# mauruszach/multimodal_diffusion

Hardware: AMD Instinct MI355X
Metric: denoising steps/sec @256x256 multimodal-cond batch=32 (higher is better)
Workload: dtype f32 via 3xbf16 split operands (6-term products, f32 accumulate; fp32-level error); 1 GPU; C3: 256x256 audio->video CFG denoising step (cond+null MMDiT d512 L8 H8 + noise head + DDIM), 384+37 tokens, batch 32 per GPU, DDIM 50 steps, guidance 3.5; global_batch=32, sampler_steps=50, parallelism=dp1, launch=eager, matmul=bf16x3, attn=default, cfg_halves=one stacked 2B batch, one stream

## Files before the change

multimodal_diffusion_amd/csrc/avd_common.h:

```cpp
#pragma once
#include <hip/hip_runtime.h>
#include <stdint.h>
#include <stdio.h>
#include <stdarg.h>
#include <atomic>

#include "../../include/avdiff_hip.h"

namespace avd {

int set_error(int code, const char* fmt, ...);

#define AVD_REQUIRE(cond, code, ...)                       \
    do {                                                   \
        if (!(cond)) return avd::set_error((code), __VA_ARGS__); \
    } while (0)

#define AVD_CHECK_LAUNCH(name)                                                          \
    do {                                                                                \
        hipError_t e__ = hipGetLastError();                                             \
        if (e__ != hipSuccess)                                                          \
            return avd::set_error(AVD_ELAUNCH, "%s: %s", (name), hipGetErrorString(e__)); \
    } while (0)

// ... 99 lines not shown
                if (fabsf(a) < __builtin_inff()) { h = (h & 0xffff8000u) | 0x7f7fu; ra = a - bf16_lo(h); } else ra = 0.f;
            }
            if ((h & 0x7fff0000u) == 0x7f800000u) {
                if (fabsf(b) < __builtin_inff()) { h = (h & 0x8000ffffu) | 0x7f7f0000u; rb = b - bf16_hi(h); } else rb = 0.f;
            }
        }
        const unsigned int m = pk_bf16(ra, rb);
        const float sa = ra - bf16_lo(m), sb = rb - bf16_hi(m);
        H[e] = h;
        Mi[e] = m;
        Lo[e] = pk_bf16(sa, sb);
    }
}

template <bool RANGE_CHECK = true>
__device__ __forceinline__ void store_split8(unsigned char* img, int64_t r, int k, int K, const float* v) {
    u32x4 H, Mi, Lo;
    split8<RANGE_CHECK>(v, H, Mi, Lo);
    const int rr = (int)(r & 127), half = (k >> 3) & 1;
    unsigned char* dst = img + ((r >> 7) * (K >> 4) + (k >> 4)) * (int64_t)S3_CHUNK + rr * 32 + ((half ^ ((rr >> 4) & 1)) << 4);
    *reinterpret_cast<u32x4*>(dst) = H;
    *reinterpret_cast<u32x4*>(dst + S3_PLANE) = Mi;
    *reinterpret_cast<u32x4*>(dst + 2 * S3_PLANE) = Lo;
}

typedef _Float16 f16x8 __attribute__((ext_vector_type(8)));
typedef _Float16 f16x2 __attribute__((ext_vector_type(2)));

__device__ __forceinline__ unsigned int pk_f16(float a, float b) {
    const f32x2 v = {a, b};
    return __builtin_bit_cast(unsigned int, __builtin_convertvector(v, f16x2));
}
__device__ __forceinline__ f32x2 unpk_f16(unsigned int p) { return __builtin_convertvector(__builtin_bit_cast(f16x2, p), f32x2); }

__device__ __forceinline__ void split8_h2(const float* v, float s, u32x4& H, u32x4& L) {
#pragma unroll
    for (int e = 0; e < 4; ++e) {
        const float a = v[2 * e] * s, b = v[2 * e + 1] * s;
        const unsigned int h = pk_f16(a, b);
        const f32x2 u = unpk_f16(h);
        H[e] = h;
        L[e] = pk_f16(a - u[0], b - u[1]);
    }
}
__device__ __forceinline__ void store_split8_h2(unsigned char* img, int64_t r, int k, int K, const float* v, float s) {
    u32x4 H, L;
// ... 72 lines not shown
extern int g_attn_pipe;
extern int g_s3_m16;
extern int g_s3_w128;
extern int g_s3_rt4;
extern int g_s3_deep4;
extern int g_s3_rt;
extern int g_vae_lat;
extern int g_vae_fold;
extern int g_codec_mfma;
extern int g_cfg_rows;
extern int g_s3_sn, g_s3_super4, g_s3_super8;
extern int g_s3_tile;
extern thread_local bool t_s3_two_streams;
int gemm_bf16x3_qkv3(const void* A3, const void* W3, const float* bias, void* img, int64_t M, int tokens, int heads, int K, float qscale,
                     int terms, hipStream_t st, float ab_scale = 1.f, float c_scale = 1.f, const float* ss_in = nullptr, float eps = 0.f);
int64_t qkv3_bytes(int B, int N, int H);
int64_t attn_fp8_ws_bytes(int B, int N, int H);
int attn_fp8(const void* qkv3, void* ws, int64_t ws_bytes, float* out, void* out3, int B, int N, int H, int n_query, hipStream_t st,
             int img_terms = 6, float img_scale = 1.f, float out_scale = 1.f);
int attn_bf16x3(const void* qkv3, float* out, void* out3, int B, int N, int H, int n_query, int terms, hipStream_t st,
                float img_scale = 1.f, float out_scale = 1.f, int out_tokens = 0);
int gemm_bf16x3(const void* A3, const void* W3, const float* bias, const float* R, float* C, void* C3, int64_t M, int N, int K,
                int act, int terms, hipStream_t st, float ab_scale = 1.f, float c_scale = 1.f, const float* ss_in = nullptr, float eps = 0.f,
                float* ss_out = nullptr, const float* gamma = nullptr, int r_seg = 0, int r_stride = 0);
bool gemm_bf16x3_resmap_supported(int terms);
bool gemm_bf16x3_rownorm_supported(int N, int terms);
extern int g_s3_splitk;
int gemm_bf16x3_splitk_slices(int64_t M, int N, int K, int terms);
int64_t gemm_bf16x3_splitk_ws_floats(int64_t M, int N, int ns);
constexpr int kS3SplitKMax = 4;
int64_t gemm_bf16x3_splitk_ws_max_floats(int64_t M, int N, int K);
int gemm_bf16x3_splitk(const void* A3, const void* W3, const float* bias, const float* R, float* C, void* C3, float* ss, int64_t M, int N,
                       int K, int terms, int ns, float* part, hipStream_t st);

}
```

multimodal_diffusion_amd/csrc/composite.hip:

```cpp
#include "avd_common.h"

#include <limits.h>
#include <stdlib.h>

#include <string.h>
#include <map>
#include <mutex>
#include <string>
#include <utility>
#include <vector>

namespace avd {

static thread_local char g_err[512] = "";

int set_error(int code, const char* fmt, ...) {
    va_list ap;
    va_start(ap, fmt);
    vsnprintf(g_err, sizeof(g_err), fmt, ap);
    va_end(ap);
    return code;
}

int LdsAttr::ensure(const void* kern, int lds_bytes, const char* what) {
// ... 119 lines not shown
    for (int l = 0; l < w->n_layers; ++l)
        if (!w->blocks[l].in_proj_weight3n || !w->blocks[l].fc1_weight3n) return false;
    return true;
}
static bool core_use_split_fold(const avd_core_weights* w) { return !g_no_fold && core_split_fold_capable(w); }

static bool core_split_rownorm_capable(const avd_core_weights* w) {
    return w->norm_kind == 0 && w->split_terms == 3 && gemm_bf16x3_rownorm_supported(w->d, 3);
}
static bool core_use_split_rownorm(const avd_core_weights* w) { return !g_no_fold && core_split_rownorm_capable(w); }

static bool core_use_fold(const avd_core_weights* w) {
    if (g_no_fold || w->norm_kind != 0) return false;
    if (!gemm_f32_fold_supported(3 * w->d, w->d) || !gemm_f32_fold_supported(w->d, w->d) ||
        !gemm_f32_fold_supported(w->mlp_hidden, w->d) || !gemm_f32_fold_supported(w->d, w->mlp_hidden))
        return false;
    for (int l = 0; l < w->n_layers; ++l)
        if (!w->blocks[l].in_proj_weight_n || !w->blocks[l].fc1_weight_n) return false;
    return true;
}

static int g_core_trim = 1;
static int64_t core_trim_floats(const avd_core_weights* w, int B, int N) { return (int64_t)B * N * w->d; }

static int64_t core_split_wide_bytes(const avd_core_weights* w, int B, int N) {
    const int64_t qkv3 = qkv3_bytes(B, N, w->n_heads), fc1 = split3_bytes((int64_t)B * N, w->mlp_hidden);
    return qkv3 > fc1 ? qkv3 : fc1;
}

static int64_t core_ws_bytes(const avd_core_weights* w, int B, int N) {
    const int64_t M = (int64_t)B * N;
    const int wide = 3 * w->d > w->mlp_hidden ? 3 * w->d : w->mlp_hidden;
    int64_t fp32_path = align_up(M * w->d * 4) + align_up(M * wide * 4) + 2 * align_up(M * (w->d / 32 + 1) * 4) +
                        align_up(gemm_f32_splitk_ws_max_floats(M, w->d, w->mlp_hidden) * 4);
    if (!core_split_capable(w, M)) return fp32_path;
    const int64_t wide_b = core_split_wide_bytes(w, B, N);
    const int64_t f8_b = w->attn_mode == 1 ? attn_fp8_ws_bytes(B, N, w->n_heads) : 0;
    const int64_t fold_b = core_split_fold_capable(w) ? align_up(split3_bytes(M, w->d)) + align_up(M * (w->d / 64) * 4)
                         : core_split_rownorm_capable(w) ? align_up(split3_bytes(M, w->d)) : 0;
    const int64_t sk_b = core_split_fold_capable(w) ? align_up(gemm_bf16x3_splitk_ws_max_floats(M, w->d, w->mlp_hidden) * 4) : 0;
    const int64_t trim_b = core_split_fold_capable(w) ? align_up(core_trim_floats(w, B, N) * 4) : 0;
    const int64_t split_path = align_up(wide_b) + align_up(split3_bytes(M, w->d)) + align_up(f8_b) + fold_b + sk_b + trim_b;
    return split_path > fp32_path ? split_path : fp32_path;
}

static int check_core(const avd_core_weights* w) {
    AVD_REQUIRE(w && w->blocks && w->final_norm_scale, AVD_EINVAL, "core: null weight table");
    AVD_REQUIRE(w->d > 0 && w->n_layers > 0 && w->n_heads > 0 && w->mlp_hidden > 0, AVD_EINVAL, "core: bad dims");
    AVD_REQUIRE(w->d % w->n_heads == 0, AVD_EINVAL, "core: d_model %d not divisible by n_heads %d", w->d, w->n_heads);
    AVD_REQUIRE(w->attn_mode == 0 || w->attn_mode == 1, AVD_EINVAL, "core: attn_mode must be 0 (follow the matmul mode) or 1 (fp8)");
    AVD_REQUIRE(w->norm_kind == 0 || w->norm_kind == 1, AVD_EINVAL, "core: norm_kind must be 0 (RMSNorm) or 1 (LayerNorm)");
    AVD_REQUIRE(w->d / w->n_heads == 64, AVD_EUNSUPPORTED, "core: head_dim %d unsupported (64 only)", w->d / w->n_heads);
    AVD_REQUIRE(w->d % 4 == 0 && w->mlp_hidden % 4 == 0, AVD_EUNSUPPORTED, "core: widths must be multiples of 4");
    AVD_REQUIRE(w->split_terms == 0 || w->split_terms == 6 || w->split_terms == 9 || w->split_terms == 1 || w->split_terms == 3, AVD_EINVAL,
                "core: split_terms must be 0/6 (default), 9 (strict), 1 (plain bf16) or 3 (f16x2), got %d", w->split_terms);
    if (w->split_terms == 3) {
        for (int l = 0; l < w->n_layers; ++l)
            for (int i = 0; i < 8; ++i) {
                const float s = w->blocks[l].f16x2_scale[i];
                AVD_REQUIRE(s > 0.f && s < __builtin_inff(), AVD_EINVAL, "core: blocks[%d].f16x2_scale[%d] must be positive and finite", l, i);
            }
    }
    return AVD_OK;
}
// ... 22 lines not shown
    const float scale = 1.0f / sqrtf((float)(d / H));
    const float* cur = x;
    AVD_REQUIRE(!(w->attn_mode == 1 && (kpm || w->norm_kind != 0)), AVD_EUNSUPPORTED,
                "core: attn_mode 1 (fp8 attention) cannot be combined with a key_padding_mask or norm_kind 1 (LayerNorm)");
    AVD_REQUIRE(!(w->attn_mode == 1 && !core_use_split(w, M)), AVD_EUNSUPPORTED,
                "core: attn_mode 1 (fp8 attention) reads the q|k|v image of the split-operand projections, which these weights / shapes "
                "do not take (every block needs its *_weight3 images; 3 d, d and mlp_hidden must be multiples of 256, d of 16)");
    if (!kpm && core_use_split(w, M)) {
        const int terms = w->split_terms;
        Carver cs{static_cast<char*>(ws), 0, ws_bytes};
        const int64_t wide_b = core_split_wide_bytes(w, B, N);
        float* qkv = cs.take((wide_b + 3) / 4);
        void* wide3 = qkv;
        void* hs = cs.take((split3_bytes(M, d) + 3) / 4);
        const int64_t f8_b = w->attn_mode == 1 ? attn_fp8_ws_bytes(B, N, H) : 0;
        float* f8w = cs.take((f8_b + 3) / 4);
        if (core_use_split_fold(w)) {
            void* hx = cs.take((split3_bytes(M, d) + 3) / 4);
            float* ss = cs.take(M * (d / 64));
            const int ns = gemm_bf16x3_splitk_slices(M, d, hid, terms);
            float* part = ns ? cs.take(gemm_bf16x3_splitk_ws_floats(M, d, ns)) : nullptr;
            const bool trim = g_core_trim && out_row0 == 0 && n_out_rows < N && w->attn_mode == 0 && gemm_bf16x3_resmap_supported(terms);
            float* yc = cs.take(core_trim_floats(w, B, N));
            const bool fused = g_mlp_fused && !ns && mlp_bf16x3_supported(d, hid, terms) && gemm_bf16x3_resmap_supported(terms);
            AVD_REQUIRE(cs.ok, AVD_EWORKSPACE, "core: workspace carve %lld > %lld bytes", (long long)cs.used, (long long)cs.cap);
            if (int rc = split3_rows_f32(cur, rd, hx, M, d, st, 0.f, ss)) return rc;
            for (int l = 0; l < w->n_layers; ++l) {
                const avd_block_weights& b = w->blocks[l];
                const bool last = l == w->n_layers - 1;
                const int nq = (last && out_row0 == 0) ? n_out_rows : N;
                if (last && trim) {
                    const int64_t Mc = (int64_t)B * nq;
                    if (int rc = gemm_bf16x3_qkv3(hx, b.in_proj_weight3n, b.in_proj_bias, qkv, M, N, H, d, scale * 1.4426950408889634f, terms, st,
                                                  1.f, 1.f, ss, w->norm_eps)) return rc;
                    if (int rc = attn_bf16x3(qkv, nullptr, hs, B, N, H, nq, terms, st, 1.f, 1.f, nq)) return rc;
                    if (int rc = gemm_bf16x3(hs, b.out_proj_weight3, b.out_proj_bias, cur, yc, hx, Mc, d, d, AVD_ACT_NONE, terms, st, 1.f, 1.f,
                                             nullptr, 0.f, ss, nullptr, nq, N)) return rc;
                    if (fused) {
                        if (int rc = mlp_bf16x3(hx, b.fc1_weight3n, b.fc1_bias, b.fc2_weight3, b.fc2_bias, ss, w->norm_eps, yc, yc, nullptr, nullptr, Mc,
                                                d, hid, st)) return rc;
                    } else {
                        if (int rc = gemm_bf16x3(hx, b.fc1_weight3n, b.fc1_bias, nullptr, nullptr, wide3, Mc, hid, d, AVD_ACT_GELU, terms, st, 1.f, 1.f,
                                                 ss, w->norm_eps)) return rc;
                        if (ns) {
                            if (int rc = gemm_bf16x3_splitk(wide3, b.fc2_weight3, b.fc2_bias, yc, yc, nullptr, nullptr, Mc, d, hid, terms, ns, part,
                                                            st)) return rc;
                        } else {
                            if (int rc = gemm_bf16x3(wide3, b.fc2_weight3, b.fc2_bias, yc, yc, nullptr, Mc, d, hid, AVD_ACT_NONE, terms, st)) return rc;
                        }
                    }
                    return rmsnorm_f32(yc, rd, w->final_norm_scale, y, RowMap{d, nq, (int64_t)N * d}, Mc, d, w->norm_eps, st);
                }
                if (int rc = gemm_bf16x3_qkv3(hx, b.in_proj_weight3n, b.in_proj_bias, qkv, M, N, H, d, scale * 1.4426950408889634f, terms, st,
                                              1.f, 1.f, ss, w->norm_eps)) return rc;
                if (w->attn_mode == 1) {
                    if (int rc = attn_fp8(qkv, f8w, f8_b, nullptr, hs, B, N, H, nq, st, terms, 1.f, 1.f)) return rc;
                } else {
                    if (int rc = attn_bf16x3(qkv, nullptr, hs, B, N, H, nq, terms, st, 1.f, 1.f)) return rc;
                }
                if (int rc = gemm_bf16x3(hs, b.out_proj_weight3, b.out_proj_bias, cur, y, hx, M, d, d, AVD_ACT_NONE, terms, st, 1.f, 1.f, nullptr,
                                         0.f, ss)) return rc;
                cur = y;
                if (fused) {
                    if (int rc = mlp_bf16x3(hx, b.fc1_weight3n, b.fc1_bias, b.fc2_weight3, b.fc2_bias, ss, w->norm_eps, y, y, last ? nullptr : hx,
                                            last ? nullptr : ss, M, d, hid, st)) return rc;
                    continue;
                }
                if (int rc = gemm_bf16x3(hx, b.fc1_weight3n, b.fc1_bias, nullptr, nullptr, wide3, M, hid, d, AVD_ACT_GELU, terms, st, 1.f, 1.f, ss,
                                         w->norm_eps)) return rc;
                if (ns) {
                    if (int rc = gemm_bf16x3_splitk(wide3, b.fc2_weight3, b.fc2_bias, y, y, last ? nullptr : hx, last ? nullptr : ss, M, d, hid,
                                                    terms, ns, part, st)) return rc;
                } else if (last) {
                    if (int rc = gemm_bf16x3(wide3, b.fc2_weight3, b.fc2_bias, y, y, nullptr, M, d, hid, AVD_ACT_NONE, terms, st)) return rc;
                } else {
                    if (int rc = gemm_bf16x3(wide3, b.fc2_weight3, b.fc2_bias, y, y, hx, M, d, hid, AVD_ACT_NONE, terms, st, 1.f, 1.f, nullptr, 0.f,
                                             ss)) return rc;
                }
            }
            return rmsnorm_f32(y, rd, w->final_norm_scale, y, rd, M, d, w->norm_eps, st);
        }
        const bool rown = core_use_split_rownorm(w);
        void* hn = rown ? cs.take((split3_bytes(M, d) + 3) / 4) : hs;
        AVD_REQUIRE(cs.ok, AVD_EWORKSPACE, "core: workspace carve %lld > %lld bytes", (long long)cs.used, (long long)cs.cap);
        for (int l = 0; l < w->n_layers; ++l) {
            const avd_block_weights& b = w->blocks[l];
            const bool last = l == w->n_layers - 1;
            const int nq = (last && out_row0 == 0) ? n_out_rows : N;
            const bool h2 = terms == 3;
            const float* fs = b.f16x2_scale;
            const float s_n1 = h2 ? fs[4] : 0.f, s_qkv = h2 ? fs[5] : 1.f, s_n2 = h2 ? fs[6] : 0.f, s_fc1 = h2 ? fs[7] : 1.f;
            const float w_in = h2 ? fs[0] : 1.f, w_out = h2 ? fs[1] : 1.f, w_fc1 = h2 ? fs[2] : 1.f, w_fc2 = h2 ? fs[3] : 1.f;
            if (!rown || l == 0)
                if (int rc = rmsnorm_split3_f32(cur, b.norm1_scale, hn, M, d, w->norm_eps, st, s_n1)) return rc;
            if (int rc = gemm_bf16x3_qkv3(hn, b.in_proj_weight3, b.in_proj_bias, qkv, M, N, H, d, scale * 1.4426950408889634f, terms, st,
                                          h2 ? s_n1 * w_in : 1.f, s_qkv)) return rc;
            if (w->attn_mode == 1) {
                if (int rc = attn_fp8(qkv, f8w, f8_b, nullptr, hs, B, N, H, nq, st, terms, s_qkv, s_qkv)) return rc;
            } else {
                if (int rc = attn_bf16x3(qkv, nullptr, hs, B, N, H, nq, terms, st, s_qkv, s_qkv)) return rc;
// ... 288 lines not shown
extern "C" const char* avd_last_error(void) { return g_err; }

constexpr int kNoExcept = INT_MIN;
struct TuneKey { const char* key; const char* env; int* var; int lo, hi; bool boolean; int except = kNoExcept; };
static const TuneKey kTuneKeys[] = {
    {"s3_tile", "AVD_S3_TILE", &g_s3_tile, INT_MIN, INT_MAX, false},
    {"s3_m16", "AVD_S3_M16", &g_s3_m16, INT_MIN, INT_MAX, false},
    {"s3_rt", "AVD_S3_RT", &g_s3_rt, INT_MIN, INT_MAX, false},
    {"s3_rt4", "AVD_S3_RT4", &g_s3_rt4, 0, 8, false, 1},
    {"s3_deep4", "AVD_S3_DEEP4", &g_s3_deep4, INT_MIN, INT_MAX, true},
    {"s3_w128", "AVD_S3_W128", &g_s3_w128, INT_MIN, INT_MAX, false},
    {"s3_splitk", "AVD_S3_SPLITK", &g_s3_splitk, 0, kS3SplitKMax, false},
    {"s3_stagger", "AVD_S3_STAGGER", &g_s3_stagger, INT_MIN, INT_MAX, false},
    {"cfg_rows", "AVD_CFG_ROWS", &g_cfg_rows, INT_MIN, INT_MAX, true},
    {"vae_lat", "AVD_VAE_LAT", &g_vae_lat, INT_MIN, INT_MAX, true},
    {"vae_fold", "AVD_VAE_FOLD", &g_vae_fold, INT_MIN, INT_MAX, true},
    {"codec_mfma", "AVD_CODEC_MFMA", &g_codec_mfma, INT_MIN, INT_MAX, true},
    {"s3_sn", "AVD_S3_SN", &g_s3_sn, INT_MIN, INT_MAX, false},
    {"s3_super4", "AVD_S3_SUPER4", &g_s3_super4, INT_MIN, INT_MAX, false},
    {"s3_super8", "AVD_S3_SUPER8", &g_s3_super8, INT_MIN, INT_MAX, false},
    {"attn_pipe", "AVD_ATTN_PIPE", &g_attn_pipe, INT_MIN, INT_MAX, false},
    {"attn_m16", "AVD_ATTN_M16", &g_attn_m16, INT_MIN, INT_MAX, false},
    {"core_trim", "AVD_CORE_TRIM", &g_core_trim, INT_MIN, INT_MAX, true},
    {"mlp_fused", "AVD_MLP_FUSED", &g_mlp_fused, INT_MIN, INT_MAX, false},
    {"gemm_tile", "AVD_GEMM_TILE", &g_gemm_force_tile, INT_MIN, INT_MAX, false},
    {"gemm_stages", "AVD_GEMM_STAGES", &g_gemm_stages, INT_MIN, INT_MAX, false},
    {"gemm_splitk", "AVD_GEMM_SPLITK", &g_gemm_splitk, 0, kGemmSplitKMax, false},
    {"s3_min_rows", "AVD_S3_MIN_ROWS", &g_s3_min_rows, INT_MIN, INT_MAX, false},
    {"no_fold", "AVD_NO_FOLD", &g_no_fold, INT_MIN, INT_MAX, true},
};
static void tune_store(const TuneKey& t, int64_t value) { *t.var = t.boolean ? value != 0 : (int)value; }
[[maybe_unused]] static const bool g_tune_env_applied = [] {
    for (const TuneKey& t : kTuneKeys)
        if (const char* e = getenv(t.env)) {
            const long long v = atoll(e);
            tune_store(t, v < t.lo ? t.lo : v > t.hi ? t.hi : v);
        }
    return true;
}();

extern "C" int avd_tune_set(const char* key, int64_t value) {
    AVD_REQUIRE(key, AVD_EINVAL, "tune_set: null key");
    for (const TuneKey& t : kTuneKeys) {
        if (strcmp(key, t.key)) continue;
        AVD_REQUIRE(value >= t.lo && value <= t.hi && value != t.except, AVD_EINVAL, "tune_set: %s does not take %lld", key, (long long)value);
        tune_store(t, value);
// ... 273 lines not shown
```

multimodal_diffusion_amd/csrc/gemm_bf16x3.hip:

```cpp
#include "avd_common.h"
#include "s3_common.h"

#include <stdlib.h>
#include <optional>
#include <type_traits>

namespace avd {


template <bool F16>
__global__ __launch_bounds__(256) void split3_kernel(const float* __restrict__ x, RowMap xm, unsigned char* __restrict__ out,
                                                     int64_t rows, int64_t rows_pad, int K, float s, float* __restrict__ ss) {
    const int64_t i = (int64_t)blockIdx.x * 256 + threadIdx.x;
    const int per_row = K >> 3;
    if (i >= rows_pad * per_row) return;
    const int64_t r = i / per_row;
    const int k = (int)(i % per_row) * 8;
    float v[8] = {0.f, 0.f, 0.f, 0.f, 0.f, 0.f, 0.f, 0.f};
    if (r < rows) {
        const float* xr = x + xm.off(r) + k;
        *reinterpret_cast<f32x4*>(v) = *reinterpret_cast<const f32x4*>(xr);
        *reinterpret_cast<f32x4*>(v + 4) = *reinterpret_cast<const f32x4*>(xr + 4);
    }
    if constexpr (F16) store_split8_h2(out, r, k, K, v, s);
// ... 226 lines not shown
                if constexpr (EPI == S3_EPI_QKV3) {
#pragma unroll
                    for (int e = 0; e < 8; ++e) v[e] = fmaf(F16 ? v[e] * g.ab_inv : v[e], rinv, bv[j][cg][e]) * mul;
                    if (S3_ROW_OK(m)) {
                        const int c = 4 * j + 2 * cg + hi;
                        unsigned char* dst = qrow + ((c ^ qsw) << 4);
                        if constexpr (F16) {
                            u32x4 Hh, Lo;
                            split8_h2(v, g.c_scale, Hh, Lo);
                            *reinterpret_cast<u32x4*>(dst) = Hh;
                            *reinterpret_cast<u32x4*>(dst + 128) = Lo;
                        } else {
                            u32x4 Hh, Mi, Lo;
                            if (big) split8<true>(v, Hh, Mi, Lo);
                            else split8<false>(v, Hh, Mi, Lo);
                            *reinterpret_cast<u32x4*>(dst) = Hh;
                            *reinterpret_cast<u32x4*>(dst + 128) = Mi;
                            *reinterpret_cast<u32x4*>(dst + 256) = Lo;
                        }
                    }
                } else if constexpr (EPI == S3_EPI_RES_IMG) {
                    const int n = nbase + 32 * j + 8 * (2 * cg + hi);
                    if (m < g.M) {
                        const float* rp = g.R + m * g.N + n;
                        const f32x4 r0 = *reinterpret_cast<const f32x4*>(rp), r1 = *reinterpret_cast<const f32x4*>(rp + 4);
#pragma unroll
                        for (int e = 0; e < 8; ++e) v[e] = ((F16 ? v[e] * g.ab_inv : v[e]) + bv[j][cg][e]) + (e < 4 ? r0[e] : r1[e - 4]);
                        float* cp = g.C + m * g.N + n;
                        *reinterpret_cast<f32x4*>(cp) = f32x4{v[0], v[1], v[2], v[3]};
                        *reinterpret_cast<f32x4*>(cp + 4) = f32x4{v[4], v[5], v[6], v[7]};
                        ssq[i] += ((v[0] * v[0] + v[1] * v[1]) + (v[2] * v[2] + v[3] * v[3])) + ((v[4] * v[4] + v[5] * v[5]) + (v[6] * v[6] + v[7] * v[7]));
                        if constexpr (F16) store_split8_h2(g.C3, m, n, g.N, v, g.c_scale);
                        else if (big) store_split8<true>(g.C3, m, n, g.N, v);
                        else store_split8<false>(g.C3, m, n, g.N, v);
                    }
                } else {
                    const int n = nbase + 32 * j + 8 * (2 * cg + hi);
#pragma unroll
                    for (int e = 0; e < 8; ++e) {
                        const float t = fmaf(F16 ? v[e] * g.ab_inv : v[e], rinv, bv[j][cg][e]);
                        v[e] = EPI == S3_EPI_GELU_SPLIT ? gelu_erf(t) : t;
                    }
                    if (S3_ROW_OK(m)) {
                        if constexpr (F16) store_split8_h2(g.C3, m, n, g.N, v, g.c_scale);
                        else if (big) store_split8<true>(g.C3, m, n, g.N, v);
                        else store_split8<false>(g.C3, m, n, g.N, v);
                    }
                }
            }
    }
    if constexpr (EPI == S3_EPI_RES_IMG) {
#pragma unroll
        for (int i = 0; i < 4; ++i) {
// ... 1114 lines not shown
static int launch_s3(const S3Args& a, hipStream_t st) {
    switch (a.terms) {
        case 0: case 6: return launch_s3t<EPI, 6>(a, st);
        case 9: return launch_s3t<EPI, 9>(a, st);
        case 1: return launch_s3t<EPI, 1>(a, st);
        case 3: return launch_s3t<EPI, 3>(a, st);
        default: return set_error(AVD_EINVAL, "gemm_bf16x3: terms must be 6 (default), 9 (strict), 1 (plain bf16) or 3 (f16x2), got %d", a.terms);
    }
}

bool gemm_bf16x3_resmap_supported(int terms) { return (terms == 0 || terms == 6) && g_s3_m16 != 0; }

static S3Args s3_args(const void* A3, const void* W3, int64_t M, int N, int K, int terms) {
    S3Args a{};
    a.A = static_cast<const unsigned char*>(A3);
    a.W = static_cast<const unsigned char*>(W3);
    a.M = M, a.N = N, a.K = K, a.terms = terms;
    a.ab_inv = a.c_scale = a.ss_sqrt_d = 1.0f;
    return a;
}

int gemm_bf16x3(const void* A3, const void* W3, const float* bias, const float* R, float* C, void* C3, int64_t M, int N, int K,
                int act, int terms, hipStream_t st, float ab_scale, float c_scale, const float* ss_in, float eps, float* ss_out,
                const float* gamma, int r_seg, int r_stride) {
    AVD_REQUIRE(r_seg == 0 || (r_seg > 0 && r_stride >= r_seg && ss_out && gemm_bf16x3_resmap_supported(terms) && M < (1ll << 31)), AVD_EUNSUPPORTED,
                "gemm_bf16x3: a residual row map needs the fp32 + image residual epilogue of the six-term 16x16x32 kernels");
    AVD_REQUIRE(A3 && W3 && (C || C3), AVD_EINVAL, "gemm_bf16x3: null pointer");
    AVD_REQUIRE(!gamma || (gemm_bf16x3_rownorm_supported(N, terms) && C && C3 && R && bias && !ss_in && !ss_out && act == AVD_ACT_NONE && aligned16(gamma)),
                AVD_EUNSUPPORTED, "gemm_bf16x3: the residual + RMSNorm epilogue needs N == 512, f16x2 images, fp32 and image outputs, bias and residual");
    AVD_REQUIRE(!ss_in || (C3 && !C && K % 64 == 0), AVD_EUNSUPPORTED, "gemm_bf16x3: a folded norm needs an image output and K %% 64 == 0");
    AVD_REQUIRE(!ss_out || (C && C3 && R && bias && N % 64 == 0 && act == AVD_ACT_NONE && terms != 3), AVD_EUNSUPPORTED,
                "gemm_bf16x3: sums of squares are written by the fp32 + image residual epilogue only (bf16 planes)");
    AVD_REQUIRE(scale_ok(ab_scale) && scale_ok(c_scale), AVD_EINVAL, "gemm_bf16x3: image scales must be positive and finite");
    AVD_REQUIRE(gemm_bf16x3_supported(M, N, K), AVD_EUNSUPPORTED, "gemm_bf16x3: need N %% 256 == 0 and K %% 16 == 0 (M=%lld N=%d K=%d)",
                (long long)M, N, K);
    AVD_REQUIRE(aligned16(A3) && aligned16(W3) && aligned16(C) && aligned16(C3) && aligned16(bias) && aligned16(R), AVD_EUNSUPPORTED,
                "gemm_bf16x3: pointers must be 16-byte aligned");
    S3Args a = s3_args(A3, W3, M, N, K, terms);
    a.bias = bias, a.R = R, a.C = C, a.C3 = static_cast<unsigned char*>(C3);
    a.ab_inv = 1.0f / ab_scale, a.c_scale = c_scale;
    a.ss_in = ss_in, a.ss_out = ss_out, a.ss_sqrt_d = (float)sqrt((double)K), a.ss_eps = eps;
    a.gamma = gamma, a.r_seg = r_seg, a.r_stride = r_stride;
    if (gamma) {
        a.ss_sqrt_d = (float)sqrt((double)N);
        return launch_s3<S3_EPI_RES_NORM>(a, st);
    }
    if (C && C3) {
        AVD_REQUIRE(ss_out, AVD_EUNSUPPORTED, "gemm_bf16x3: fp32 and image output together imply the residual + sums-of-squares epilogue");
        return launch_s3<S3_EPI_RES_IMG>(a, st);
    }
    if (C3) {
        AVD_REQUIRE((act == AVD_ACT_GELU || act == AVD_ACT_NONE) && !R && bias, AVD_EUNSUPPORTED,
                    "gemm_bf16x3: image output implies bias, act NONE or GELU, no residual");
        return act == AVD_ACT_GELU ? launch_s3<S3_EPI_GELU_SPLIT>(a, st) : launch_s3<S3_EPI_SPLIT>(a, st);
    }
    AVD_REQUIRE(act == AVD_ACT_NONE, AVD_EUNSUPPORTED, "gemm_bf16x3: fp32 output supports act NONE only");
    if (R) {
        if ((terms == 0 || terms == 6) && g_s3_m16 && bias) return launch_s3<S3_EPI_RES_IMG>(a, st);
        return launch_s3<S3_EPI_RES>(a, st);
    }
    return launch_s3<S3_EPI_BIAS>(a, st);
}

template <bool IMG>
__global__ __launch_bounds__(256) void splitk_reduce_kernel(const float* __restrict__ part, int ns, const float* __restrict__ bias,
// ... 141 lines not shown
```

multimodal_diffusion_amd/csrc/mlp_bf16x3.hip:

```cpp
#include "avd_common.h"
#include "s3_common.h"

#include <stdlib.h>

namespace avd {

constexpr int ML_BM = 128, ML_HC = 64, ML_D = 512;
constexpr int ML_H = 4 * S3_CHUNK;
constexpr int ML_S1 = S3_CHUNK + 3 * ML_HC * 32;
constexpr int ML_NS1 = 3;
constexpr int ML_S2 = 3 * ML_D * 32;
constexpr int ML_LDS = ML_H + 2 * ML_S2;
static_assert(ML_NS1 * ML_S1 <= 2 * ML_S2, "phase-1 ring fits the stage area");

struct MlpArgs {
    const unsigned char* X;
    const unsigned char* W1;
    const float* b1;
    const unsigned char* W2;
    const float* ss_in;
    int hidden;
    float sqrt_d, eps;
    S3Args epi;
};
// ... 167 lines not shown
            };
            auto ldb = [&](bf16x8 (&dst)[8], int type) {
#pragma unroll
                for (int j = 0; j < 8; ++j) dst[j] = *reinterpret_cast<const bf16x8*>(ws + plane_of(type, ML_D * 32) + j * 512 + ((j & 1) ? base_o : base_e));
            };
            ML_SB();
            lda(ahl, T_HL); ldb(bx, T_LH); ML_SB();
            lda(ahm, T_HM); ldb(by, T_MH); ML_SB();
            mm2(ahl, bx, false); ML_SB();
            ldb(bx, T_HM); ML_SB();
            mm2(ahm, by, false); ML_SB();
            mm2(ahm, bx, last); ML_SB();
        };
        for (int kt = 0; kt < 3; ++kt) phase2_step(false, kt);
        phase2_step(true, 3);
    }
#undef ML_SB
#undef ML_BARRIER
    int lane_e = lane;
    asm volatile("s_nop 15\n\ts_nop 15"
                 : "+v"(lane_e), "+a"(acc2[0][6][0]), "+a"(acc2[0][6][1]), "+a"(acc2[0][6][2]), "+a"(acc2[0][6][3]), "+a"(acc2[1][6][0]),
                   "+a"(acc2[1][6][1]), "+a"(acc2[1][6][2]), "+a"(acc2[1][6][3]), "+a"(acc2[0][7][0]), "+a"(acc2[0][7][1]), "+a"(acc2[0][7][2]),
                   "+a"(acc2[0][7][3]), "+a"(acc2[1][7][0]), "+a"(acc2[1][7][1]), "+a"(acc2[1][7][2]), "+a"(acc2[1][7][3]));
    s3_epilogue_img16<S3_EPI_RES_IMG, 8>(g.epi, acc2[0], m0, wave * 128, lane_e);
    s3_epilogue_img16<S3_EPI_RES_IMG, 8>(g.epi, acc2[1], m0, wave * 128 + 64, lane_e);
}

int g_mlp_fused = 0;

bool mlp_bf16x3_supported(int d, int hidden, int terms) { return d == ML_D && hidden > 0 && hidden % 128 == 0 && (terms == 0 || terms == 6); }

int mlp_bf16x3(const void* X3, const void* W1n3, const float* b1, const void* W23, const float* b2, const float* ss_in, float eps,
               const float* R, float* C, void* C3, float* ss_out, int64_t M, int d, int hidden, hipStream_t st) {
    AVD_REQUIRE(X3 && W1n3 && b1 && W23 && b2 && ss_in && R && C, AVD_EINVAL, "mlp_bf16x3: null pointer");
    AVD_REQUIRE((C3 != nullptr) == (ss_out != nullptr), AVD_EINVAL, "mlp_bf16x3: the image and the sums of squares come together");
    AVD_REQUIRE(mlp_bf16x3_supported(d, hidden, 6), AVD_EUNSUPPORTED, "mlp_bf16x3: d must be 512 and hidden a multiple of 128 (d=%d hidden=%d)", d, hidden);
    AVD_REQUIRE(M > 0 && (M + ML_BM - 1) / ML_BM < (1ll << 31), AVD_EINVAL, "mlp_bf16x3: bad row count");
    AVD_REQUIRE(aligned16(X3) && aligned16(W1n3) && aligned16(W23) && aligned16(b1) && aligned16(b2) && aligned16(ss_in) && aligned16(R) &&
                    aligned16(C) && aligned16(C3), AVD_EUNSUPPORTED, "mlp_bf16x3: pointers must be 16-byte aligned");
    static LdsAttr attr;
    if (int rc = attr.ensure(reinterpret_cast<const void*>(mlp_bf16x3_kernel), ML_LDS, "mlp_bf16x3")) return rc;
    MlpArgs a{};
    a.X = static_cast<const unsigned char*>(X3);
    a.W1 = static_cast<const unsigned char*>(W1n3);
    a.b1 = b1;
    a.W2 = static_cast<const unsigned char*>(W23);
    a.ss_in = ss_in;
    a.hidden = hidden;
// ... 21 lines not shown
```

multimodal_diffusion_amd/csrc/s3_common.h:

```cpp
#pragma once
#include "avd_common.h"

namespace avd {

#define AVD_LDS_PTR(p) ((__attribute__((address_space(3))) void*)(p))
#define AVD_GLB_PTR(p) ((const __attribute__((address_space(1))) void*)(p))

enum { S3_EPI_BIAS = 0, S3_EPI_RES = 2, S3_EPI_GELU_SPLIT = 3, S3_EPI_QKV3 = 4, S3_EPI_SPLIT = 5, S3_EPI_RES_IMG = 6, S3_EPI_RES_NORM = 7,
       S3_EPI_BIAS_REG = 8 };

struct S3Args {
    const unsigned char* A;
    const unsigned char* W;
    const float* bias;
    const float* R;
    float* C;
    unsigned char* C3;
    int64_t M;
    int N, K, nbn, sm, sn;
    int tokN, tokNpad, heads;
    float qscale;
    int stagger;
    int first_gen;
    int terms;
    float ab_inv, c_scale;
    const float* ss_in;
    float* ss_out;
    float ss_sqrt_d, ss_eps;
    const float* gamma;
    int r_seg, r_stride;
#ifdef AVD_S3_STAMPS
    unsigned long long* dbg;
#endif
};

#ifdef AVD_S3_STAMPS
#define S3_T() __builtin_amdgcn_s_memtime()
#define S3_RT() __builtin_amdgcn_s_memrealtime()
#define S3_DBG(i, v) do { if (threadIdx.x == 0) g.dbg[(size_t)blockIdx.x * 16 + (i)] = (v); } while (0)
#else
#define S3_T() 0ull
#define S3_RT() 0ull
#define S3_DBG(i, v) do { } while (0)
#endif

__device__ __forceinline__ void s3_block_of(const S3Args& g, int nbm, int& bm, int& bn) {
    const int b = blockIdx.x, nwg = gridDim.x, q = nwg >> 3, r = nwg & 7, x = b & 7;
    const int wg = (x < r ? x * (q + 1) : r * (q + 1) + (x - r) * q) + (b >> 3);
    const int per_row = g.sm * g.nbn;
    const int srow = wg / per_row, rem = wg - srow * per_row;
    const int left = nbm - srow * g.sm, h = left < g.sm ? left : g.sm;
    const int per_st = h * g.sn;
    const int sc = rem / per_st, rem2 = rem - sc * per_st;
    bm = srow * g.sm + rem2 / g.sn;
    bn = sc * g.sn + rem2 % g.sn;
}

template <int N> __device__ __forceinline__ void wait_vm() {
    static_assert(N >= 0 && N < 64, "vmcnt range");
    __builtin_amdgcn_s_waitcnt(0x0f70 | (N & 15) | ((N >> 4) << 14));
}

#ifdef AVD_LAB_NOSTORE
#define S3_ROW_OK(m) ((m) < g.M && __float_as_uint(v[0]) == 0x7fc12345u)
#else
#define S3_ROW_OK(m) ((m) < g.M)
#endif

typedef float f32x4t __attribute__((ext_vector_type(4)));

__device__ __forceinline__ f32x4t mma16x16(bf16x8 a, bf16x8 b, f32x4t c) { return __builtin_amdgcn_mfma_f32_16x16x32_bf16(a, b, c, 0, 0, 0); }

template <int EPI, int RT = 8>
__device__ __forceinline__ void s3_epilogue_img16(const S3Args& g, f32x4t (&acc)[8][4], int64_t mwave0, int nbase, int lane) {
    const int l15 = lane & 15, kq = lane >> 4;
    bool big = EPI == S3_EPI_RES_IMG;
    if constexpr (EPI != S3_EPI_RES_IMG && EPI != S3_EPI_BIAS_REG) {
        float amax = 0.f;
#pragma unroll
        for (int i = 0; i < 8; ++i) {
            float a = 0.f;
#pragma unroll
            for (int j = 0; j < 4; ++j)
#pragma unroll
                for (int r = 0; r < 4; ++r) a = fmaxf(a, fabsf(acc[i][j][r]));
            if (mwave0 + 16 * i + l15 < g.M) amax = fmaxf(amax, a);
        }
        float bmax = 0.f;
#pragma unroll
        for (int e = 0; e < 64; e += 4) {
            const f32x4 b4 = *reinterpret_cast<const f32x4*>(g.bias + nbase + e);
            bmax = fmaxf(fmaxf(bmax, fmaxf(fabsf(b4[0]), fabsf(b4[1]))), fmaxf(fabsf(b4[2]), fabsf(b4[3])));
        }
        big = __any(!(amax < 1.2676506e30f) || !(bmax < 1.2676506e30f) || !(fabsf(g.qscale) < 1.0e6f));
    }
    float bv[4][8];
// ... 57 lines not shown
            if constexpr (EPI == S3_EPI_QKV3) {
#pragma unroll
                for (int e = 0; e < 8; ++e) v[e] = fmaf(v[e], rinv, bv[j][e]) * mul;
                if (S3_ROW_OK(m)) {
                    const int c = 2 * j + (kq >> 1);
                    unsigned char* dst = qrow + ((c ^ qsw) << 4);
                    u32x4 Hh, Mi, Lo;
                    if (big) split8<true>(v, Hh, Mi, Lo);
                    else split8<false>(v, Hh, Mi, Lo);
                    *reinterpret_cast<u32x4*>(dst) = Hh;
                    *reinterpret_cast<u32x4*>(dst + 128) = Mi;
                    *reinterpret_cast<u32x4*>(dst + 256) = Lo;
                }
            } else if constexpr (EPI == S3_EPI_BIAS_REG) {
                if (S3_ROW_OK(m)) {
#pragma unroll
                    for (int e = 0; e < 8; ++e) v[e] += bv[j][e];
                    float* cp = g.C + m * g.N + n;
                    *reinterpret_cast<f32x4*>(cp) = f32x4{v[0], v[1], v[2], v[3]};
                    *reinterpret_cast<f32x4*>(cp + 4) = f32x4{v[4], v[5], v[6], v[7]};
                }
            } else if constexpr (EPI == S3_EPI_RES_IMG) {
                if (S3_ROW_OK(m)) {
                    const float* rp = g.R + rrow * g.N + n;
                    const f32x4 r0 = *reinterpret_cast<const f32x4*>(rp), r1 = *reinterpret_cast<const f32x4*>(rp + 4);
#pragma unroll
                    for (int e = 0; e < 8; ++e) v[e] = (v[e] + bv[j][e]) + (e < 4 ? r0[e] : r1[e - 4]);
                    float* cp = g.C + m * g.N + n;
                    *reinterpret_cast<f32x4*>(cp) = f32x4{v[0], v[1], v[2], v[3]};
                    *reinterpret_cast<f32x4*>(cp + 4) = f32x4{v[4], v[5], v[6], v[7]};
                    ssq += ((v[0] * v[0] + v[1] * v[1]) + (v[2] * v[2] + v[3] * v[3])) + ((v[4] * v[4] + v[5] * v[5]) + (v[6] * v[6] + v[7] * v[7]));
                    if (g.C3) store_split8<true>(g.C3, m, n, g.N, v);
                }
            } else {
#pragma unroll
                for (int e = 0; e < 8; ++e) {
                    const float t = fmaf(v[e], rinv, bv[j][e]);
                    v[e] = EPI == S3_EPI_GELU_SPLIT ? gelu_erf(t) : t;
                }
                if (S3_ROW_OK(m)) {
                    if (big) store_split8<true>(g.C3, m, n, g.N, v);
                    else store_split8<false>(g.C3, m, n, g.N, v);
                }
            }
        }
        if constexpr (EPI == S3_EPI_RES_IMG) {
            const float tot = ssq + __shfl_xor(ssq, 32, 64);
            if (kq < 2 && m < g.M && g.ss_out) g.ss_out[m * (g.N >> 6) + (nbase >> 6)] = tot;
        }
    }
}

}
// ... 1 lines not shown
```

Before: 119.0 steps/s.

## Read residual from split bf16x3 image instead of fp32 stream, lazy fp32 store

The residual epilogue now reconstructs the residual from the already-written three-plane bf16 image (H+Mi+Lo), falling back to the fp32 buffer only for chunks with tiny magnitudes where the split loses precision. The fp32 output store is also skipped (c_lazy) unless the chunk contains tiny values, so subsequent layers read from the image. This is meant to cut fp32 residual read/write traffic per layer, at the cost of extra workspace for a separate image buffer in the trimmed last layer and some per-chunk branching.

```diff
diff --git a/multimodal_diffusion_amd/csrc/avd_common.h b/multimodal_diffusion_amd/csrc/avd_common.h
--- a/multimodal_diffusion_amd/csrc/avd_common.h
+++ b/multimodal_diffusion_amd/csrc/avd_common.h
@@ -145,6 +145,20 @@
     *reinterpret_cast<u32x4*>(dst) = H;
     *reinterpret_cast<u32x4*>(dst + S3_PLANE) = Mi;
     *reinterpret_cast<u32x4*>(dst + 2 * S3_PLANE) = Lo;
+}
+
+__device__ __forceinline__ void load_split8(const unsigned char* img, int64_t r, int k, int K, float* v) {
+#pragma clang fp contract(off)
+    const int rr = (int)(r & 127), half = (k >> 3) & 1;
+    const unsigned char* src = img + ((r >> 7) * (K >> 4) + (k >> 4)) * (int64_t)S3_CHUNK + rr * 32 + ((half ^ ((rr >> 4) & 1)) << 4);
+    const u32x4 H = *reinterpret_cast<const u32x4*>(src);
+    const u32x4 Mi = *reinterpret_cast<const u32x4*>(src + S3_PLANE);
+    const u32x4 Lo = *reinterpret_cast<const u32x4*>(src + 2 * S3_PLANE);
+#pragma unroll
+    for (int e = 0; e < 4; ++e) {
+        v[2 * e] = bf16_lo(H[e]) + (bf16_lo(Mi[e]) + bf16_lo(Lo[e]));
+        v[2 * e + 1] = bf16_hi(H[e]) + (bf16_hi(Mi[e]) + bf16_hi(Lo[e]));
+    }
 }
 
 typedef _Float16 f16x8 __attribute__((ext_vector_type(8)));
@@ -263,7 +277,8 @@
                 float img_scale = 1.f, float out_scale = 1.f, int out_tokens = 0);
 int gemm_bf16x3(const void* A3, const void* W3, const float* bias, const float* R, float* C, void* C3, int64_t M, int N, int K,
                 int act, int terms, hipStream_t st, float ab_scale = 1.f, float c_scale = 1.f, const float* ss_in = nullptr, float eps = 0.f,
-                float* ss_out = nullptr, const float* gamma = nullptr, int r_seg = 0, int r_stride = 0);
+                float* ss_out = nullptr, const float* gamma = nullptr, int r_seg = 0, int r_stride = 0, const void* R3 = nullptr,
+                bool c_lazy = false);
 bool gemm_bf16x3_resmap_supported(int terms);
 bool gemm_bf16x3_rownorm_supported(int N, int terms);
 extern int g_s3_splitk;
diff --git a/multimodal_diffusion_amd/csrc/composite.hip b/multimodal_diffusion_amd/csrc/composite.hip
--- a/multimodal_diffusion_amd/csrc/composite.hip
+++ b/multimodal_diffusion_amd/csrc/composite.hip
@@ -165,6 +165,7 @@
 
 static int g_core_trim = 1;
 static int64_t core_trim_floats(const avd_core_weights* w, int B, int N) { return (int64_t)B * N * w->d; }
+static int g_s3_res_img = 1;
 
 static int64_t core_split_wide_bytes(const avd_core_weights* w, int B, int N) {
     const int64_t qkv3 = qkv3_bytes(B, N, w->n_heads), fc1 = split3_bytes((int64_t)B * N, w->mlp_hidden);
@@ -182,7 +183,7 @@
     const int64_t fold_b = core_split_fold_capable(w) ? align_up(split3_bytes(M, w->d)) + align_up(M * (w->d / 64) * 4)
                          : core_split_rownorm_capable(w) ? align_up(split3_bytes(M, w->d)) : 0;
     const int64_t sk_b = core_split_fold_capable(w) ? align_up(gemm_bf16x3_splitk_ws_max_floats(M, w->d, w->mlp_hidden) * 4) : 0;
-    const int64_t trim_b = core_split_fold_capable(w) ? align_up(core_trim_floats(w, B, N) * 4) : 0;
+    const int64_t trim_b = core_split_fold_capable(w) ? align_up(core_trim_floats(w, B, N) * 4) + align_up(split3_bytes(M, w->d)) : 0;
     const int64_t split_path = align_up(wide_b) + align_up(split3_bytes(M, w->d)) + align_up(f8_b) + fold_b + sk_b + trim_b;
     return split_path > fp32_path ? split_path : fp32_path;
 }
@@ -251,8 +252,11 @@
             float* part = ns ? cs.take(gemm_bf16x3_splitk_ws_floats(M, d, ns)) : nullptr;
             const bool trim = g_core_trim && out_row0 == 0 && n_out_rows < N && w->attn_mode == 0 && gemm_bf16x3_resmap_supported(terms);
             float* yc = cs.take(core_trim_floats(w, B, N));
+            void* hxc = cs.take((split3_bytes(M, d) + 3) / 4);
             const bool fused = g_mlp_fused && !ns && mlp_bf16x3_supported(d, hid, terms) && gemm_bf16x3_resmap_supported(terms);
             AVD_REQUIRE(cs.ok, AVD_EWORKSPACE, "core: workspace carve %lld > %lld bytes", (long long)cs.used, (long long)cs.cap);
+            const bool res_img = g_s3_res_img && !ns && !fused;
+            const bool res_img_fc2 = res_img && gemm_bf16x3_resmap_supported(terms);
             if (int rc = split3_rows_f32(cur, rd, hx, M, d, st, 0.f, ss)) return rc;
             for (int l = 0; l < w->n_layers; ++l) {
                 const avd_block_weights& b = w->blocks[l];
@@ -263,19 +267,21 @@
                     if (int rc = gemm_bf16x3_qkv3(hx, b.in_proj_weight3n, b.in_proj_bias, qkv, M, N, H, d, scale * 1.4426950408889634f, terms, st,
                                                   1.f, 1.f, ss, w->norm_eps)) return rc;
                     if (int rc = attn_bf16x3(qkv, nullptr, hs, B, N, H, nq, terms, st, 1.f, 1.f, nq)) return rc;
-                    if (int rc = gemm_bf16x3(hs, b.out_proj_weight3, b.out_proj_bias, cur, yc, hx, Mc, d, d, AVD_ACT_NONE, terms, st, 1.f, 1.f,
-                                             nullptr, 0.f, ss, nullptr, nq, N)) return rc;
+                    void* hc = res_img ? hxc : hx;
+                    if (int rc = gemm_bf16x3(hs, b.out_proj_weight3, b.out_proj_bias, cur, yc, hc, Mc, d, d, AVD_ACT_NONE, terms, st, 1.f, 1.f,
+                                             nullptr, 0.f, ss, nullptr, nq, N, res_img ? hx : nullptr, res_img_fc2)) return rc;
                     if (fused) {
-                        if (int rc = mlp_bf16x3(hx, b.fc1_weight3n, b.fc1_bias, b.fc2_weight3, b.fc2_bias, ss, w->norm_eps, yc, yc, nullptr, nullptr, Mc,
+                        if (int rc = mlp_bf16x3(hc, b.fc1_weight3n, b.fc1_bias, b.fc2_weight3, b.fc2_bias, ss, w->norm_eps, yc, yc, nullptr, nullptr, Mc,
                                                 d, hid, st)) return rc;
                     } else {
-                        if (int rc = gemm_bf16x3(hx, b.fc1_weight3n, b.fc1_bias, nullptr, nullptr, wide3, Mc, hid, d, AVD_ACT_GELU, terms, st, 1.f, 1.f,
+                        if (int rc = gemm_bf16x3(hc, b.fc1_weight3n, b.fc1_bias, nullptr, nullptr, wide3, Mc, hid, d, AVD_ACT_GELU, terms, st, 1.f, 1.f,
                                                  ss, w->norm_eps)) return rc;
                         if (ns) {
                             if (int rc = gemm_bf16x3_splitk(wide3, b.fc2_weight3, b.fc2_bias, yc, yc, nullptr, nullptr, Mc, d, hid, terms, ns, part,
                                                             st)) return rc;
                         } else {
-                            if (int rc = gemm_bf16x3(wide3, b.fc2_weight3, b.fc2_bias, yc, yc, nullptr, Mc, d, hid, AVD_ACT_NONE, terms, st)) return rc;
+                            if (int rc = gemm_bf16x3(wide3, b.fc2_weight3, b.fc2_bias, yc, yc, nullptr, Mc, d, hid, AVD_ACT_NONE, terms, st, 1.f, 1.f,
+                                                     nullptr, 0.f, nullptr, nullptr, 0, 0, res_img_fc2 ? hc : nullptr)) return rc;
                         }
                     }
                     return rmsnorm_f32(yc, rd, w->final_norm_scale, y, RowMap{d, nq, (int64_t)N * d}, Mc, d, w->norm_eps, st);
@@ -288,7 +294,7 @@
                     if (int rc = attn_bf16x3(qkv, nullptr, hs, B, N, H, nq, terms, st, 1.f, 1.f)) return rc;
                 }
                 if (int rc = gemm_bf16x3(hs, b.out_proj_weight3, b.out_proj_bias, cur, y, hx, M, d, d, AVD_ACT_NONE, terms, st, 1.f, 1.f, nullptr,
-                                         0.f, ss)) return rc;
+                                         0.f, ss, nullptr, 0, 0, res_img ? hx : nullptr, last ? res_img_fc2 : res_img)) return rc;
                 cur = y;
                 if (fused) {
                     if (int rc = mlp_bf16x3(hx, b.fc1_weight3n, b.fc1_bias, b.fc2_weight3, b.fc2_bias, ss, w->norm_eps, y, y, last ? nullptr : hx,
@@ -301,10 +307,11 @@
                     if (int rc = gemm_bf16x3_splitk(wide3, b.fc2_weight3, b.fc2_bias, y, y, last ? nullptr : hx, last ? nullptr : ss, M, d, hid,
                                                     terms, ns, part, st)) return rc;
                 } else if (last) {
-                    if (int rc = gemm_bf16x3(wide3, b.fc2_weight3, b.fc2_bias, y, y, nullptr, M, d, hid, AVD_ACT_NONE, terms, st)) return rc;
+                    if (int rc = gemm_bf16x3(wide3, b.fc2_weight3, b.fc2_bias, y, y, nullptr, M, d, hid, AVD_ACT_NONE, terms, st, 1.f, 1.f, nullptr,
+                                             0.f, nullptr, nullptr, 0, 0, res_img_fc2 ? hx : nullptr)) return rc;
                 } else {
                     if (int rc = gemm_bf16x3(wide3, b.fc2_weight3, b.fc2_bias, y, y, hx, M, d, hid, AVD_ACT_NONE, terms, st, 1.f, 1.f, nullptr, 0.f,
-                                             ss)) return rc;
+                                             ss, nullptr, 0, 0, res_img ? hx : nullptr, res_img)) return rc;
                 }
             }
             return rmsnorm_f32(y, rd, w->final_norm_scale, y, rd, M, d, w->norm_eps, st);
@@ -639,6 +646,7 @@
     {"attn_pipe", "AVD_ATTN_PIPE", &g_attn_pipe, INT_MIN, INT_MAX, false},
     {"attn_m16", "AVD_ATTN_M16", &g_attn_m16, INT_MIN, INT_MAX, false},
     {"core_trim", "AVD_CORE_TRIM", &g_core_trim, INT_MIN, INT_MAX, true},
+    {"s3_res_img", "AVD_S3_RES_IMG", &g_s3_res_img, INT_MIN, INT_MAX, true},
     {"mlp_fused", "AVD_MLP_FUSED", &g_mlp_fused, INT_MIN, INT_MAX, false},
     {"gemm_tile", "AVD_GEMM_TILE", &g_gemm_force_tile, INT_MIN, INT_MAX, false},
     {"gemm_stages", "AVD_GEMM_STAGES", &g_gemm_stages, INT_MIN, INT_MAX, false},
diff --git a/multimodal_diffusion_amd/csrc/gemm_bf16x3.hip b/multimodal_diffusion_amd/csrc/gemm_bf16x3.hip
--- a/multimodal_diffusion_amd/csrc/gemm_bf16x3.hip
+++ b/multimodal_diffusion_amd/csrc/gemm_bf16x3.hip
@@ -272,13 +272,11 @@
                 } else if constexpr (EPI == S3_EPI_RES_IMG) {
                     const int n = nbase + 32 * j + 8 * (2 * cg + hi);
                     if (m < g.M) {
-                        const float* rp = g.R + m * g.N + n;
-                        const f32x4 r0 = *reinterpret_cast<const f32x4*>(rp), r1 = *reinterpret_cast<const f32x4*>(rp + 4);
-#pragma unroll
-                        for (int e = 0; e < 8; ++e) v[e] = ((F16 ? v[e] * g.ab_inv : v[e]) + bv[j][cg][e]) + (e < 4 ? r0[e] : r1[e - 4]);
-                        float* cp = g.C + m * g.N + n;
-                        *reinterpret_cast<f32x4*>(cp) = f32x4{v[0], v[1], v[2], v[3]};
-                        *reinterpret_cast<f32x4*>(cp + 4) = f32x4{v[4], v[5], v[6], v[7]};
+                        float rv[8];
+                        s3_res_chunk(g, m, n, rv);
+#pragma unroll
+                        for (int e = 0; e < 8; ++e) v[e] = ((F16 ? v[e] * g.ab_inv : v[e]) + bv[j][cg][e]) + rv[e];
+                        s3_res_store_c(g, m, n, v);
                         ssq[i] += ((v[0] * v[0] + v[1] * v[1]) + (v[2] * v[2] + v[3] * v[3])) + ((v[4] * v[4] + v[5] * v[5]) + (v[6] * v[6] + v[7] * v[7]));
                         if constexpr (F16) store_split8_h2(g.C3, m, n, g.N, v, g.c_scale);
                         else if (big) store_split8<true>(g.C3, m, n, g.N, v);
@@ -1439,7 +1437,12 @@
 
 int gemm_bf16x3(const void* A3, const void* W3, const float* bias, const float* R, float* C, void* C3, int64_t M, int N, int K,
                 int act, int terms, hipStream_t st, float ab_scale, float c_scale, const float* ss_in, float eps, float* ss_out,
-                const float* gamma, int r_seg, int r_stride) {
+                const float* gamma, int r_seg, int r_stride, const void* R3, bool c_lazy) {
+    AVD_REQUIRE(!R3 || (R && C && bias && !gamma && terms != 3 && act == AVD_ACT_NONE && aligned16(R3) &&
+                        ((C3 && ss_out) || (!C3 && gemm_bf16x3_resmap_supported(terms)))),
+                AVD_EUNSUPPORTED, "gemm_bf16x3: a residual image needs the residual + image epilogue of the bf16-plane kernels");
+    AVD_REQUIRE(!c_lazy || (R3 && C3), AVD_EINVAL, "gemm_bf16x3: c_lazy needs the residual image and an image output");
+    AVD_REQUIRE(!(R3 && r_seg > 0 && R3 == C3), AVD_EINVAL, "gemm_bf16x3: mapped residual rows cannot be read from the image being written");
     AVD_REQUIRE(r_seg == 0 || (r_seg > 0 && r_stride >= r_seg && ss_out && gemm_bf16x3_resmap_supported(terms) && M < (1ll << 31)), AVD_EUNSUPPORTED,
                 "gemm_bf16x3: a residual row map needs the fp32 + image residual epilogue of the six-term 16x16x32 kernels");
     AVD_REQUIRE(A3 && W3 && (C || C3), AVD_EINVAL, "gemm_bf16x3: null pointer");
@@ -1458,6 +1461,7 @@
     a.ab_inv = 1.0f / ab_scale, a.c_scale = c_scale;
     a.ss_in = ss_in, a.ss_out = ss_out, a.ss_sqrt_d = (float)sqrt((double)K), a.ss_eps = eps;
     a.gamma = gamma, a.r_seg = r_seg, a.r_stride = r_stride;
+    a.R3 = static_cast<const unsigned char*>(R3), a.c_lazy = c_lazy;
     if (gamma) {
         a.ss_sqrt_d = (float)sqrt((double)N);
         return launch_s3<S3_EPI_RES_NORM>(a, st);
diff --git a/multimodal_diffusion_amd/csrc/mlp_bf16x3.hip b/multimodal_diffusion_amd/csrc/mlp_bf16x3.hip
--- a/multimodal_diffusion_amd/csrc/mlp_bf16x3.hip
+++ b/multimodal_diffusion_amd/csrc/mlp_bf16x3.hip
@@ -213,8 +213,8 @@
                  : "+v"(lane_e), "+a"(acc2[0][6][0]), "+a"(acc2[0][6][1]), "+a"(acc2[0][6][2]), "+a"(acc2[0][6][3]), "+a"(acc2[1][6][0]),
                    "+a"(acc2[1][6][1]), "+a"(acc2[1][6][2]), "+a"(acc2[1][6][3]), "+a"(acc2[0][7][0]), "+a"(acc2[0][7][1]), "+a"(acc2[0][7][2]),
                    "+a"(acc2[0][7][3]), "+a"(acc2[1][7][0]), "+a"(acc2[1][7][1]), "+a"(acc2[1][7][2]), "+a"(acc2[1][7][3]));
-    s3_epilogue_img16<S3_EPI_RES_IMG, 8>(g.epi, acc2[0], m0, wave * 128, lane_e);
-    s3_epilogue_img16<S3_EPI_RES_IMG, 8>(g.epi, acc2[1], m0, wave * 128 + 64, lane_e);
+    s3_epilogue_img16<S3_EPI_RES_IMG, 8, false>(g.epi, acc2[0], m0, wave * 128, lane_e);
+    s3_epilogue_img16<S3_EPI_RES_IMG, 8, false>(g.epi, acc2[1], m0, wave * 128 + 64, lane_e);
 }
 
 int g_mlp_fused = 0;
diff --git a/multimodal_diffusion_amd/csrc/s3_common.h b/multimodal_diffusion_amd/csrc/s3_common.h
--- a/multimodal_diffusion_amd/csrc/s3_common.h
+++ b/multimodal_diffusion_amd/csrc/s3_common.h
@@ -29,6 +29,8 @@
     float ss_sqrt_d, ss_eps;
     const float* gamma;
     int r_seg, r_stride;
+    const unsigned char* R3;
+    int c_lazy;
 #ifdef AVD_S3_STAMPS
     unsigned long long* dbg;
 #endif
@@ -71,7 +73,32 @@
 
 __device__ __forceinline__ f32x4t mma16x16(bf16x8 a, bf16x8 b, f32x4t c) { return __builtin_amdgcn_mfma_f32_16x16x32_bf16(a, b, c, 0, 0, 0); }
 
-template <int EPI, int RT = 8>
+constexpr float kResTinyStore = 0x1p-96f, kResTinyLoad = 0x1p-100f;
+__device__ __forceinline__ bool s3_chunk_below(const float* v, float thr) {
+    float a = fabsf(v[0]);
+#pragma unroll
+    for (int e = 1; e < 8; ++e) a = fminf(a, fabsf(v[e]));
+    return a < thr;
+}
+template <bool IMG = true>
+__device__ __forceinline__ void s3_res_chunk(const S3Args& g, int64_t r, int n, float* rv) {
+    if (IMG && g.R3) {
+        load_split8(g.R3, r, n, g.N, rv);
+        if (!s3_chunk_below(rv, kResTinyLoad)) return;
+    }
+    const float* rp = g.R + r * g.N + n;
+    *reinterpret_cast<f32x4*>(rv) = *reinterpret_cast<const f32x4*>(rp);
+    *reinterpret_cast<f32x4*>(rv + 4) = *reinterpret_cast<const f32x4*>(rp + 4);
+}
+template <bool IMG = true>
+__device__ __forceinline__ void s3_res_store_c(const S3Args& g, int64_t m, int n, const float* v) {
+    if (IMG && g.c_lazy && !s3_chunk_below(v, kResTinyStore)) return;
+    float* cp = g.C + m * g.N + n;
+    *reinterpret_cast<f32x4*>(cp) = f32x4{v[0], v[1], v[2], v[3]};
+    *reinterpret_cast<f32x4*>(cp + 4) = f32x4{v[4], v[5], v[6], v[7]};
+}
+
+template <int EPI, int RT = 8, bool RES3 = true>
 __device__ __forceinline__ void s3_epilogue_img16(const S3Args& g, f32x4t (&acc)[8][4], int64_t mwave0, int nbase, int lane) {
     const int l15 = lane & 15, kq = lane >> 4;
     bool big = EPI == S3_EPI_RES_IMG;
@@ -175,13 +202,11 @@
                 }
             } else if constexpr (EPI == S3_EPI_RES_IMG) {
                 if (S3_ROW_OK(m)) {
-                    const float* rp = g.R + rrow * g.N + n;
-                    const f32x4 r0 = *reinterpret_cast<const f32x4*>(rp), r1 = *reinterpret_cast<const f32x4*>(rp + 4);
-#pragma unroll
-                    for (int e = 0; e < 8; ++e) v[e] = (v[e] + bv[j][e]) + (e < 4 ? r0[e] : r1[e - 4]);
-                    float* cp = g.C + m * g.N + n;
-                    *reinterpret_cast<f32x4*>(cp) = f32x4{v[0], v[1], v[2], v[3]};
-                    *reinterpret_cast<f32x4*>(cp + 4) = f32x4{v[4], v[5], v[6], v[7]};
+                    float rv[8];
+                    s3_res_chunk<RES3>(g, rrow, n, rv);
+#pragma unroll
+                    for (int e = 0; e < 8; ++e) v[e] = (v[e] + bv[j][e]) + rv[e];
+                    s3_res_store_c<RES3>(g, m, n, v);
                     ssq += ((v[0] * v[0] + v[1] * v[1]) + (v[2] * v[2] + v[3] * v[3])) + ((v[4] * v[4] + v[5] * v[5]) + (v[6] * v[6] + v[7] * v[7]));
                     if (g.C3) store_split8<true>(g.C3, m, n, g.N, v);
                 }
```

Result: no change. 119.9 steps/s, median of 6 (+0.7%).
